# JoshEngels/RangeFilteredANN

Measured on AMD Instinct MI355X. Metric: QPS @ recall@10>=0.95, window fraction 2^-3, higher is better.
Workload: dtype f32

## Files before the change

### include/wann.h

```cpp
#ifndef WANN_H
#define WANN_H

#include <stdint.h>

#ifdef __cplusplus
extern "C" {
#endif

#define WANN_ABI_VERSION 5
#define WANN_MAX_DEGREE 128

enum { WANN_OK = 0, WANN_ERR_INVALID = 1, WANN_ERR_NO_DEVICE = 2, WANN_ERR_HIP = 3, WANN_ERR_IO = 4,
       WANN_ERR_UNSUPPORTED = 5 };

enum { WANN_METRIC_L2 = 0, WANN_METRIC_MIPS = 1 };
enum { WANN_DTYPE_F32 = 0, WANN_DTYPE_U8 = 1, WANN_DTYPE_I8 = 2, WANN_DTYPE_F16 = 3, WANN_DTYPE_BF16 = 5 };
enum {
  WANN_KIND_PREFILTER = 0,
  WANN_KIND_POSTFILTER = 1,
  WANN_KIND_TREE_PREFILTER = 2,
  WANN_KIND_TREE_VAMANA = 3,
  WANN_KIND_SUPER = 4
};

// ... 82 lines not shown
typedef struct {
  int64_t queries;
  int64_t unproven;
  int64_t rescued;
  int64_t groups;
  int64_t tiles;
  int64_t passes;
  int64_t handover_bytes;
} wann_dense_window_counters;
int wann_get_dense_window_counters(const wann_index *index, wann_dense_window_counters *out);

int64_t wann_set_exact_windows(wann_index *index, int64_t max_points);
typedef struct {
  int64_t queries;
  int64_t dense_queries;
  int64_t unproven;
  int64_t rescued;
  int64_t passes;
  int64_t rows_scanned;
} wann_exact_window_counters;
int wann_get_exact_window_counters(const wann_index *index, wann_exact_window_counters *out);

int64_t wann_num_points(const wann_index *index);
int64_t wann_dim(const wann_index *index);
int64_t wann_num_levels(const wann_index *index);
int64_t wann_level_size(const wann_index *index, int64_t level);
int wann_partition_range(const wann_index *index, int64_t level, int64_t idx, int64_t *start, int64_t *end);
int wann_partition_graph(const wann_index *index, int64_t level, int64_t idx, int32_t *rows, int64_t cap_rows,
                         int64_t max_degree);
int64_t wann_max_degree(const wann_index *index);
int64_t wann_device_bytes(const wann_index *index);

int wann_rows_fp16_exact(const float *rows, int64_t n, int64_t d);
int wann_set_half_rows(wann_index *index, int on);
int wann_half_rows(const wann_index *index);
int64_t wann_half_rows_bytes(const wann_index *index);
int wann_last_half_rows(const wann_index *index);
int wann_rows_u8_exact(const float *rows, int64_t n, int64_t d);
int64_t wann_byte_row_position(int64_t element);
int wann_set_byte_rows(wann_index *index, int on);
int wann_byte_rows(const wann_index *index);
int64_t wann_byte_rows_bytes(const wann_index *index);
int wann_last_byte_rows(const wann_index *index);
int wann_set_scan_rows(wann_index *index, int on);
int wann_scan_rows(const wann_index *index);
int wann_last_scan_rows(const wann_index *index);
int wann_num_replicas(const wann_index *index);

int wann_gather_layout(int64_t nq, int world, int shard, int64_t *lo, int64_t *count, int64_t *cap);
int wann_batch_search_allgather(wann_index *index, const void *queries, const float *ranges, int64_t nq, const char *method,
                                const wann_query_params *qp, int32_t **d_planes, int64_t *cap);

int wann_build_cache_shard(int kind, int metric, int dtype, const void *points, int64_t n, int64_t d,
                           const float *labels, int32_t cutoff, double split_factor,
                           double shift_factor, const wann_build_params *bp, int shard, int nshards,
                           int build_threads);

int wann_raw_beam_search(int metric, const float *points, int64_t n, int64_t d,
                         const int32_t *graph_rows , int64_t maxdeg,
                         int64_t subset_start, int64_t subset_n, const float *queries, int64_t nq,
                         const int64_t *query_ids, int64_t beam, int64_t limit,
                         int64_t degree_limit, int32_t *out_ids ,
                         float *out_dists , int32_t *out_sizes ,
                         int64_t *out_hops , int64_t *out_dist_cmps , int device);
int wann_raw_beam_search_typed(int metric, int dtype, const void *points, int64_t n, int64_t d,
                               const int32_t *graph_rows , int64_t maxdeg,
// ... 21 lines not shown
```

### rangefilteredann_amd/csrc/wann_abi.cpp

```cpp
#include "wann_host_internal.h"

struct wann_index::AsyncLane {
  Workspace ws;
  hipStream_t stream = nullptr, side = nullptr;
  hipEvent_t ready = nullptr;
  wann_counters last{};
  int last_store = kStoreRows;
  struct Job {
    const float *q, *r;
    int64_t nq, base;
    std::string method;
    wann_query_params qp;
    uint32_t *ids;
    float *dists;
    int64_t ticket;
    Tuning tune;
  };
  std::thread th;
  std::mutex m;
  std::condition_variable cv;
  bool has_job = false, busy = false, stop = false;
  Job job{};
  int64_t finished = -1;
  int rc = WANN_OK;
// ... 671 lines not shown
  return WANN_OK;
}
int64_t wann_max_degree(const wann_index *I) { return I ? I->H.spec.R : -1; }
int64_t wann_device_bytes(const wann_index *I) { return I ? I->device_bytes : -1; }

int wann_rows_fp16_exact(const float *rows, int64_t n, int64_t d) {
  if (n <= 0 || d <= 0) return 1;
  if (!rows) return 0;
  return rows_fp16_exact(rows, n, d, d, 0) ? 1 : 0;
}

int wann_set_half_rows(wann_index *I, int on) {
  if (!I) return -fail(WANN_ERR_INVALID, "null argument");
  int now;
  {
    std::lock_guard<std::mutex> lk(I->tune_mu);
    now = I->half_rows_on = on != 0 && I->d_half.p != nullptr;
  }
  for (auto &R : I->replicas) {
    std::lock_guard<std::mutex> lr(R->tune_mu);
    R->half_rows_on = on != 0 && R->d_half.p != nullptr;
  }
  return now;
}

int wann_half_rows(const wann_index *I) {
  if (!I) return 0;
  wann_index *M = const_cast<wann_index *>(I);
  std::lock_guard<std::mutex> lk(M->tune_mu);
  return I->half_rows_on ? 1 : 0;
}

int64_t wann_half_rows_bytes(const wann_index *I) { return I ? (int64_t)I->d_half.bytes() : -1; }
int wann_last_half_rows(const wann_index *I) { return I ? I->last_half_rows.load() : 0; }

int wann_rows_u8_exact(const float *rows, int64_t n, int64_t d) {
  if (n <= 0 || d <= 0) return 1;
  if (!rows) return 0;
  return rows_u8_exact(rows, n, d, d, 0) ? 1 : 0;
}

int64_t wann_byte_row_position(int64_t element) { return element < 0 ? -1 : u8_row_position(element); }

int wann_set_byte_rows(wann_index *I, int on) {
  if (!I) return -fail(WANN_ERR_INVALID, "null argument");
  int now;
  {
    std::lock_guard<std::mutex> lk(I->tune_mu);
    now = I->byte_rows_on = on != 0 && I->d_bytes.p != nullptr;
  }
  for (auto &R : I->replicas) {
    std::lock_guard<std::mutex> lr(R->tune_mu);
    R->byte_rows_on = on != 0 && R->d_bytes.p != nullptr;
  }
  return now;
}

int wann_byte_rows(const wann_index *I) {
  if (!I) return 0;
  wann_index *M = const_cast<wann_index *>(I);
  std::lock_guard<std::mutex> lk(M->tune_mu);
  return I->byte_rows_on ? 1 : 0;
}

int64_t wann_byte_rows_bytes(const wann_index *I) { return I ? (int64_t)I->d_bytes.bytes() : -1; }
int wann_last_byte_rows(const wann_index *I) { return I ? I->last_byte_rows.load() : 0; }
// ... 44 lines not shown
```

### rangefilteredann_amd/csrc/wann_build.cpp

```cpp
#include "wann_build.h"
#include "wann_device.h"
#include "wann_bf16.h"
#include "wann_half.h"

#include <algorithm>
#include <atomic>
#include <climits>
#include <cmath>
#include <condition_variable>
#include <cstdio>
#include <cstdlib>
#include <cstring>
#include <mutex>
#include <stdexcept>
#include <sys/stat.h>
#include <thread>
#include <unistd.h>
#include <chrono>

namespace wann {

namespace {
class WorkerPool {
 public:
// ... 128 lines not shown
    if (!exact.load(std::memory_order_relaxed)) return;
    const float *p = rows + r * stride;
    for (int64_t j = 0; j < d; j++) {
      uint32_t u = 0, v = 1;
      if (p[j] >= 0.f && p[j] <= 255.f) {
        const float back = (float)(uint8_t)p[j];
        memcpy(&u, p + j, 4);
        memcpy(&v, &back, 4);
      }
      if (u != v) {
        exact.store(false, std::memory_order_relaxed);
        return;
      }
    }
  });
  return exact.load();
}

void pack_u8_rows(const float *rows, int64_t n, int64_t d, int64_t stride, int64_t out_words, int threads, float *out) {
  parallel_for(n, threads > 0 ? threads : default_threads(), [&](int64_t r) {
    const float *src = rows + r * stride;
    uint8_t *dst = reinterpret_cast<uint8_t *>(out + r * out_words);
    for (int64_t j = 0; j < d; j++) dst[j] = (uint8_t)src[j];
  });
}

void interleave_u8_rows(float *rows, int64_t n, int64_t words, int threads) {
  if (words <= 0 || words % 8 != 0) throw std::runtime_error("interleave_u8_rows: a row is a whole number of 32-byte groups");
  parallel_for(n, threads > 0 ? threads : default_threads(), [&](int64_t r) {
    uint8_t *row = reinterpret_cast<uint8_t *>(rows + r * words);
    for (int64_t g = 0; g < words * 4; g += 32) {
      uint8_t t[32];
      for (int e = 0; e < 32; e++) t[u8_row_position(e)] = row[g + e];
      memcpy(row + g, t, 32);
    }
  });
}

static inline uint64_t mix64(uint64_t x) {
  x = (x ^ (x >> 30)) * UINT64_C(0xbf58476d1ce4e5b9);
  x = (x ^ (x >> 27)) * UINT64_C(0x94d049bb133111eb);
  return x ^ (x >> 31);
}

static inline float l2_ref_order(const float *a, const float *b, int d) {
  const int D8 = (d + 7) >> 3;
  float acc[8] = {0, 0, 0, 0, 0, 0, 0, 0};
  const bool odd = D8 & 1;
  for (int i = 0; i < D8; i++) {
    const int blk = odd ? (i == 0 ? D8 - 1 : i - 1) : i;
    const float *pa = a + 8 * blk, *pb = b + 8 * blk;
    for (int j = 0; j < 8; j++) {
      float t = pa[j] - pb[j];
      acc[j] = std::fmaf(t, t, acc[j]);
    }
  }
  return ((((((acc[0] + acc[1]) + acc[2]) + acc[3]) + acc[4]) + acc[5]) + acc[6]) + acc[7];
}

static inline float mips_ref_order(const float *p, const float *q, int d) {
  const int dv = d & ~7;
  float r = 0.f;
  for (int i = 0; i < dv; i++) {
    volatile float prod = q[i] * p[i];
    r = r + prod;
  }
// ... 622 lines not shown
```

### rangefilteredann_amd/csrc/wann_build.h

```cpp
#pragma once
#include <stdint.h>

#include <functional>
#include <string>
#include <vector>

namespace wann {

struct HostGraph {
  int64_t n = 0;
  int32_t maxdeg = 0;
  std::vector<int32_t> rows;
  int32_t *row(int64_t i) { return rows.data() + i * (maxdeg + 1); }
  const int32_t *row(int64_t i) const { return rows.data() + i * (maxdeg + 1); }
};

struct HostPart {
  int64_t start = 0, n = 0;
  float lo = 0, hi = 0;
  HostGraph g;
};

struct BuildSpec {
  int kind = 0, metric = 0;
  int dtype = 0;
  int64_t n = 0, d = 0, stride = 0;
  int32_t cutoff = 1000;
  double split_factor = 2, shift_factor = 0.5;
  int64_t R = 64, L = 500;
  double alpha = 1.0;
  std::string cache;
  int threads = 0;
};

struct HostIndex {
  BuildSpec spec;
  bool vamana_leaves = false, sorted = false;
  std::vector<float> pts;
  std::vector<float> labels;
  std::vector<uint32_t> decoding;
  std::vector<std::vector<int64_t>> offsets;
  std::vector<int64_t> sup_size, sup_shift;
  std::vector<std::vector<HostPart>> levels;
  std::vector<float> fv_sorted;
  std::vector<int32_t> fi_sorted;
};

void parallel_for(int64_t n, int threads, const std::function<void(int64_t)> &f);
int default_threads();

bool rows_fp16_exact(const float *rows, int64_t n, int64_t d, int64_t stride, int threads);
bool rows_u8_exact(const float *rows, int64_t n, int64_t d, int64_t stride, int threads);
void pack_u8_rows(const float *rows, int64_t n, int64_t d, int64_t stride, int64_t out_words, int threads, float *out);
void interleave_u8_rows(float *rows, int64_t n, int64_t words, int threads);

float host_distance(int metric, const float *p, const float *q, int d);

bool graph_file_load(const std::string &path, HostGraph &g);
bool graph_file_save(const std::string &path, const HostGraph &g);
std::string graph_file_name(const BuildSpec &s, float lo, float hi, int64_t n);

std::vector<int32_t> insertion_order(int64_t n);

void vamana_build(const float *pts, int64_t stride, int64_t d, int metric, int64_t start, int64_t n,
                  int64_t R, int64_t L, double alpha, HostGraph &g, int threads);

void build_host_index(HostIndex &H, const void *points, const float *labels, int shard = -1,
                      int nshards = 0, std::vector<HostPart *> *pending = nullptr);
void build_pending_on_host(HostIndex &H, std::vector<HostPart *> &pending);
void save_built_graphs(HostIndex &H, std::vector<HostPart *> &built, bool keep);

}
```

### rangefilteredann_amd/csrc/wann_device.h

```cpp
#pragma once
#include <stdint.h>

namespace wann {

struct PartDesc {
  int64_t row_base;
  int32_t start;
  int32_t n;
};

struct IndexView {
  const float *points;
  const float *labels;
  const uint32_t *decoding;
  const int32_t *graph;
  const PartDesc *parts;
  const float *fv_sorted;
  const int32_t *fi_sorted;
  const int64_t *wst_off;
  const int64_t *wst_ptr;
  const int64_t *level_part0;
  const int64_t *level_nb;
  const int64_t *sup_size;
  const int64_t *sup_shift;
  int64_t n;
  int32_t d, stride, rs, maxdeg, metric, kind, nlevels, cutoff, split, vamana_leaves;
  int32_t dtype;
};

constexpr bool two_byte_rows(int dtype) { return dtype == 3 || dtype == 5; }
constexpr int64_t two_byte_stride_words(int64_t d) { return ((d * 2 + 63) / 64) * 16; }

constexpr int kRowsU8Widened = 6;
constexpr int64_t u8_widened_stride_words(int64_t d) { return ((d + 63) / 64) * 16; }
constexpr int64_t u8_row_position(int64_t e) { return 32 * (e >> 5) + 16 * ((e >> 2) & 1) + 4 * ((e >> 3) & 3) + (e & 3); }
constexpr bool widened_rows(int dtype) { return two_byte_rows(dtype) || dtype == kRowsU8Widened; }

inline int query_words(const IndexView &v) { return widened_rows(v.dtype) ? ((v.d + 15) & ~15) : v.stride; }

enum { T_EMPTY = 0, T_GRAPH = 1, T_BRUTE = 2, T_BRUTE_GATHER = 3, T_PARENT = 4 };
constexpr int kTaskExactWindow = 32;
enum { M_OPTIMIZED = 0, M_THREE_SPLIT = 1, M_FENWICK = 2 };

struct Task {
  int32_t query;
  int32_t mode;
  int32_t part;
  int32_t flags;
  int64_t a, b;
  float lo, hi;
};

struct CoverCounters {
  unsigned long long queries, unproven, rescued, groups, tiles, passes, handover_bytes;
};

struct Counters {
  unsigned long long beam_searches, hops, dist_cmps, brute_rows, label_reads, unsupported;
  unsigned long long spec_searches, spec_hops, spec_dist_cmps;
  unsigned long long poll_timeouts;
  unsigned long long gemm_queries, gemm_unproven, gemm_rescued;
  unsigned long long deep_handoffs;
  unsigned long long lookaheads_used;
  unsigned long long big_searches, big_hops, packet_hops, own_scorings, prefetched_hops;
// ... 233 lines not shown
```

### rangefilteredann_amd/csrc/wann_host.cpp

```cpp
#include "wann_host_internal.h"
#include "wann_bf16.h"
#include "wann_half.h"

namespace wann_host {


thread_local std::string g_err;
int fail(int code, const std::string &msg) {
  g_err = msg;
  return code;
}

int usable_devices() {
  int n = 0;
  if (hipGetDeviceCount(&n) != hipSuccess) return 0;
  return n;
}

int hash_bits(int64_t beam) {
  return std::max<int>(10, (int)std::ceil(std::log2((double)(beam * beam))) - 2);
}

void convert_rows(const HostGraph &g, int rs, int32_t *out) {
  for (int64_t i = 0; i < g.n; i++) {
// ... 50 lines not shown
  v.maxdeg = (int32_t)s.R;
  v.rs = (int32_t)(((s.R + 15) / 16) * 16);
  v.nlevels = (int32_t)H.levels.size();

  if (two_byte_rows(s.dtype)) {
    std::vector<float> rows((size_t)s.n * v.stride, 0.f);
    parallel_for(s.n, s.threads > 0 ? s.threads : default_threads(), [&](int64_t r) {
      const float *src = H.pts.data() + r * s.stride;
      uint16_t *dst = reinterpret_cast<uint16_t *>(rows.data() + r * v.stride);
      for (int64_t j = 0; j < s.d; j++) dst[j] = float_to_two_byte(s.dtype, src[j]);
    });
    I.d_points.upload(rows);
  } else {
    I.d_points.upload(H.pts);
  }
  if (s.dtype == WANN_DTYPE_F32 && H.vamana_leaves && rows_fp16_exact(H.pts.data(), s.n, s.d, s.stride, s.threads)) {
    const int64_t hstride = ((s.d * 2 + 63) / 64) * 16;
    std::vector<float> rows;
    try {
      rows.assign((size_t)s.n * hstride, 0.f);
      I.d_half.ensure(rows.size());
    } catch (std::bad_alloc &) {
      I.d_half.release();
    } catch (HipError &) {
      (void)hipGetLastError();
      I.d_half.release();
    }
    if (I.d_half.p) {
      parallel_for(s.n, s.threads > 0 ? s.threads : default_threads(), [&](int64_t r) {
        const float *src = H.pts.data() + r * s.stride;
        uint16_t *dst = reinterpret_cast<uint16_t *>(rows.data() + r * hstride);
        for (int64_t j = 0; j < s.d; j++) dst[j] = float_to_half(src[j]);
      });
      I.d_half.upload(rows);
    }
  }
  if (s.dtype == WANN_DTYPE_F32 && H.vamana_leaves && rows_u8_exact(H.pts.data(), s.n, s.d, s.stride, s.threads)) {
    const int64_t bstride = u8_widened_stride_words(s.d);
    std::vector<float> rows;
    try {
      rows.assign((size_t)s.n * bstride, 0.f);
      I.d_bytes.ensure(rows.size());
    } catch (std::bad_alloc &) {
      I.d_bytes.release();
    } catch (HipError &) {
      (void)hipGetLastError();
      I.d_bytes.release();
    }
    if (I.d_bytes.p) {
      pack_u8_rows(H.pts.data(), s.n, s.d, s.stride, bstride, s.threads, rows.data());
      interleave_u8_rows(rows.data(), s.n, bstride, s.threads);
      I.d_bytes.upload(rows);
    }
  }
  I.d_labels.upload(H.labels);
  I.d_decoding.upload(H.decoding);
  v.points = I.d_points.p;
  v.labels = I.d_labels.p;
  v.decoding = I.d_decoding.p;
  if (s.kind == WANN_KIND_PREFILTER) {
    I.d_fv.upload(H.fv_sorted);
    I.d_fi.upload(H.fi_sorted);
    v.fv_sorted = I.d_fv.p;
    v.fi_sorted = I.d_fi.p;
  }
  int64_t rows = 0;
// ... 39 lines not shown
            for (int j = 0; j < deg; j++) {
              if (r[1 + j] < 0 || r[1 + j] >= P.n) throw std::runtime_error("graph edge out of range");
              o[j] = r[1 + j];
            }
            for (int j = deg; j < v.rs; j++) o[j] = -1;
          }
          HIP_CHECK(hipMemcpy(I.d_graph.p + (pd.row_base + r0) * v.rs, stage.data(), stage.size() * 4, hipMemcpyHostToDevice));
        }
      }
    v.graph = I.d_graph.p;
  }
  if (!H.offsets.empty()) {
    std::vector<int64_t> flat, ptr;
    for (auto &o : H.offsets) {
      ptr.push_back((int64_t)flat.size());
      flat.insert(flat.end(), o.begin(), o.end());
    }
    ptr.push_back((int64_t)flat.size());
    I.d_wst_off.upload(flat);
    I.d_wst_ptr.upload(ptr);
    v.wst_off = I.d_wst_off.p;
    v.wst_ptr = I.d_wst_ptr.p;
  }
  if (!H.sup_size.empty()) {
    I.d_sup_size.upload(H.sup_size);
    I.d_sup_shift.upload(H.sup_shift);
    v.sup_size = I.d_sup_size.p;
    v.sup_shift = I.d_sup_shift.p;
  }
  I.search_view = v;
  if (I.d_half.p) {
    I.search_view.points = I.d_half.p;
    I.search_view.stride = (int32_t)(((s.d * 2 + 63) / 64) * 16);
    I.search_view.dtype = WANN_DTYPE_F16;
    I.half_rows_on = true;
  }
  I.byte_view = v;
  if (I.d_bytes.p) {
    I.byte_view.points = I.d_bytes.p;
    I.byte_view.stride = (int32_t)u8_widened_stride_words(s.d);
    I.byte_view.dtype = kRowsU8Widened;
  }
  I.device_bytes = (int64_t)(I.d_points.bytes() + I.d_labels.bytes() + I.d_decoding.bytes() + I.d_graph.bytes() +
                             I.d_parts.bytes() + I.d_fv.bytes() + I.d_fi.bytes() + I.d_wst_off.bytes());
}

int ensure_filter_scratch(DevBuf<int32_t> &table, DevBuf<int32_t> &epoch, DevBuf<uint32_t> &seen, int64_t &layout, int slots,
                          int table_bits, int64_t seen_words, hipStream_t st, bool any_slots) {
  if (any_slots && layout > table_bits && layout < 32 && ((size_t)slots << layout) * sizeof(int32_t) <= ((size_t)20 << 30)) table_bits = (int)layout;
  const size_t need = (size_t)slots << table_bits;
  const int64_t want = any_slots ? (int64_t)table_bits : (((int64_t)slots << 8) | table_bits);
  const bool fresh = need > table.cap || (size_t)slots > epoch.cap;
  table.ensure(need);
  epoch.ensure((size_t)slots);
  seen.ensure((size_t)slots * (size_t)seen_words);
  if (fresh || layout != want) {
    HIP_CHECK(hipMemsetAsync(table.p, 0, table.cap * sizeof(int32_t), st));
    HIP_CHECK(hipMemsetAsync(epoch.p, 0, epoch.cap * sizeof(int32_t), st));
    layout = want;
  }
  return table_bits;
}

constexpr int kLdsGranule = 1280;
inline int lds_blocks_per_cu(int per_block) { return kLdsPerWorkgroup / (((per_block + kLdsGranule - 1) / kLdsGranule) * kLdsGranule); }

RoundCfg config_for(const wann_index &I, const IndexView &V, const Tuning &T, int64_t first_beam, int64_t cap, int64_t work_items, bool big_lds, bool force_table,
// ... 130 lines not shown
```

### rangefilteredann_amd/csrc/wann_kernels_body.inc

```
#include <hip/hip_runtime.h>
#include <stdint.h>

#include <algorithm>

#include "wann_device.h"
#include "wann_wave.h"

namespace wann {

#if WANN_DT == 0
#define WANN_DT_NS dt_f32
#elif WANN_DT == 1
#define WANN_DT_NS dt_u8
#elif WANN_DT == 2
#define WANN_DT_NS dt_i8
#elif WANN_DT == 3
#define WANN_DT_NS dt_f16
#elif WANN_DT == 5
#define WANN_DT_NS dt_bf16
#else
#define WANN_DT_NS dt_w8
#endif
#if WANN_DT == 3
#define WANN_DT_TPARAM , int ROWS_DT = 3
#elif WANN_DT == 5
#define WANN_DT_TPARAM , int ROWS_DT = 5
#elif WANN_DT == 6
#define WANN_DT_TPARAM , int ROWS_DT = 6
#else
#define WANN_DT_TPARAM
#endif
#ifndef WANN_MIPS_WAVES
#define WANN_MIPS_WAVES 3
#endif
namespace WANN_DT_NS {


__device__ __forceinline__ int hash_bits_dev(long long beam) {
  long long sq = beam * beam;
  int e = (sq <= 1) ? 0 : (64 - __builtin_clzll((unsigned long long)(sq - 1)));
  e -= 2;
  return e < 10 ? 10 : e;
}

__device__ __forceinline__ void la_withdraw(const SearchArgs &A, int la) {
  if (atomicExch(&A.par_done[la], 2) == 1) {
    atomicAdd(&A.ctr->spec_searches, 1ull);
    atomicAdd(&A.ctr->spec_hops, (unsigned long long)__hip_atomic_load(&A.sub_hops[la], __ATOMIC_RELAXED, __HIP_MEMORY_SCOPE_AGENT));
    atomicAdd(&A.ctr->spec_dist_cmps, (unsigned long long)__hip_atomic_load(&A.sub_cmps[la], __ATOMIC_RELAXED, __HIP_MEMORY_SCOPE_AGENT));
  }
  atomicCAS(A.dyn_list + A.next_beam[la], la, -2 - la);
}

__device__ __forceinline__ int la_slot_of(const SearchArgs &A, int t) {
  long long v = __hip_atomic_load(&A.sub_cmps[t], __ATOMIC_RELAXED, __HIP_MEMORY_SCOPE_AGENT);
  for (int spin = 0; v == -2 && spin < 4096; spin++) {
    __builtin_amdgcn_s_sleep(2);
    v = __hip_atomic_load(&A.sub_cmps[t], __ATOMIC_RELAXED, __HIP_MEMORY_SCOPE_AGENT);
  }
  return v < 0 ? -1 : (int)v;
}
// ... 1279 lines not shown
#endif
  dim3 grid(blocks), block(64 * kWavesPerBlock);
  return a.ix.metric == 1 ? launch_brute_t<1>(a, grid, block, lds, (hipStream_t)stream) : launch_brute_t<0>(a, grid, block, lds, (hipStream_t)stream);
}

}

#if WANN_DT == 0
namespace dt_u8 {
int launch_search(const SearchArgs &a, const LaunchCfg &cfg, void *stream);
int search_occupancy(const SearchArgs &a, const LaunchCfg &cfg);
int launch_brute(const BruteArgs &a, int blocks, void *stream);
}
namespace dt_i8 {
int launch_search(const SearchArgs &a, const LaunchCfg &cfg, void *stream);
int search_occupancy(const SearchArgs &a, const LaunchCfg &cfg);
int launch_brute(const BruteArgs &a, int blocks, void *stream);
}
namespace dt_f16 {
int launch_search(const SearchArgs &a, const LaunchCfg &cfg, void *stream);
int search_occupancy(const SearchArgs &a, const LaunchCfg &cfg);
int launch_brute(const BruteArgs &a, int blocks, void *stream);
}
namespace dt_bf16 {
int launch_search(const SearchArgs &a, const LaunchCfg &cfg, void *stream);
int search_occupancy(const SearchArgs &a, const LaunchCfg &cfg);
int launch_brute(const BruteArgs &a, int blocks, void *stream);
}
namespace dt_w8 {
int launch_search(const SearchArgs &a, const LaunchCfg &cfg, void *stream);
int search_occupancy(const SearchArgs &a, const LaunchCfg &cfg);
int launch_brute(const BruteArgs &a, int blocks, void *stream);
}
int search_occupancy(const SearchArgs &a, const LaunchCfg &cfg) {
  return a.ix.dtype == 1 ? dt_u8::search_occupancy(a, cfg) : a.ix.dtype == 2 ? dt_i8::search_occupancy(a, cfg)
       : a.ix.dtype == 3 ? dt_f16::search_occupancy(a, cfg) : a.ix.dtype == 5 ? dt_bf16::search_occupancy(a, cfg)
       : a.ix.dtype == kRowsU8Widened ? dt_w8::search_occupancy(a, cfg) : dt_f32::search_occupancy(a, cfg);
}
int launch_search(const SearchArgs &a, const LaunchCfg &cfg, void *stream) {
  return a.ix.dtype == 1 ? dt_u8::launch_search(a, cfg, stream) : a.ix.dtype == 2 ? dt_i8::launch_search(a, cfg, stream)
       : a.ix.dtype == 3 ? dt_f16::launch_search(a, cfg, stream) : a.ix.dtype == 5 ? dt_bf16::launch_search(a, cfg, stream)
       : a.ix.dtype == kRowsU8Widened ? dt_w8::launch_search(a, cfg, stream) : dt_f32::launch_search(a, cfg, stream);
}
int launch_brute(const BruteArgs &a, int blocks, void *stream) {
  return a.ix.dtype == 1 ? dt_u8::launch_brute(a, blocks, stream) : a.ix.dtype == 2 ? dt_i8::launch_brute(a, blocks, stream)
       : a.ix.dtype == 3 ? dt_f16::launch_brute(a, blocks, stream) : a.ix.dtype == 5 ? dt_bf16::launch_brute(a, blocks, stream)
       : a.ix.dtype == kRowsU8Widened ? dt_w8::launch_brute(a, blocks, stream) : dt_f32::launch_brute(a, blocks, stream);
}

int launch_finalize(const FinalizeArgs &a, void *stream) {
  if (a.nq == 0) return 0;
  if (a.maxt > 1) {
    const int per_wave = finalize_lds_bytes_per_wave(a.k);
    int blocks = (int)std::min<int64_t>(2048, (a.nq + kWavesPerBlock - 1) / kWavesPerBlock);
    hipLaunchKernelGGL(k_finalize_multi, dim3(blocks), dim3(64 * kWavesPerBlock), (size_t)per_wave * kWavesPerBlock,
                       (hipStream_t)stream, a);
  } else {
    int threads = 256;
    int blocks = (int)((a.nq * (int64_t)a.k + threads - 1) / threads);
    hipLaunchKernelGGL(k_finalize, dim3(blocks), dim3(threads), 0, (hipStream_t)stream, a);
  }
  return check(hipGetLastError());
}

#endif

}
```

### rangefilteredann_amd/csrc/wann_wave.h

```cpp
#pragma once
#include <hip/hip_runtime.h>
#include <stdint.h>

#include "wann_device.h"

namespace wann {

typedef unsigned long long u64;

#ifdef WANN_PHASE_PROFILE
#define WANN_PROF_PTR(p) (p)
#else
#define WANN_PROF_PTR(p) ((unsigned long long *)nullptr)
#endif

#define WANN_LIKELY(x) __builtin_expect(!!(x), 1)
#define WANN_UNLIKELY(x) __builtin_expect(!!(x), 0)

#define WAVE_SYNC()                                            \
  do {                                                         \
    __builtin_amdgcn_fence(__ATOMIC_SEQ_CST, "wavefront");     \
    __builtin_amdgcn_wave_barrier();                           \
  } while (0)

// ... 15 lines not shown
__device__ __forceinline__ T *uniptr(T *p) {
  return reinterpret_cast<T *>(uni64((long long)reinterpret_cast<uintptr_t>(p)));
}
__device__ __forceinline__ int ctz64(u64 m) { return __builtin_ctzll(m); }
__device__ __forceinline__ int popc64(u64 m) { return __builtin_popcountll(m); }
__device__ __forceinline__ u64 lanemask_lt() { return ((u64)1 << lane_id()) - 1; }

__device__ __forceinline__ int wave_ticket(int32_t *cursor) {
  int lane;
  asm volatile("v_mbcnt_lo_u32_b32 %0, -1, 0\n\tv_mbcnt_hi_u32_b32 %0, -1, %0" : "=v"(lane));
  int t = 0;
  if (lane == 0) t = atomicAdd(cursor, 1);
  return __builtin_amdgcn_readfirstlane(t);
}

__device__ __forceinline__ uint32_t fkey(float f) {
  uint32_t u = __float_as_uint(f);
  return (u & 0x80000000u) ? ~u : (u | 0x80000000u);
}
__device__ __forceinline__ float funkey(uint32_t k) {
  return __uint_as_float((k & 0x80000000u) ? (k ^ 0x80000000u) : ~k);
}

__device__ __forceinline__ u64 hash64_2(u64 x) {
  x = (x ^ (x >> 30)) * 0xbf58476d1ce4e5b9ull;
  x = (x ^ (x >> 27)) * 0x94d049bb133111ebull;
  return x ^ (x >> 31);
}

#ifndef WANN_DT
#define WANN_DT 0
#endif
#define WANN_BYTE_ROWS (WANN_DT == 1 || WANN_DT == 2)
#define WANN_HALF_ROWS (WANN_DT == 3 || WANN_DT == 5)
#define WANN_WIDENED_ROWS (WANN_HALF_ROWS || WANN_DT == 6)

#if WANN_DT == 3
typedef uint2 rowblk_t;
__device__ __forceinline__ float h2f(uint32_t bits) { return (float)__builtin_bit_cast(_Float16, (unsigned short)bits); }
__device__ __forceinline__ float4 h4_to_f4(uint2 w) {
  return make_float4(h2f(w.x & 0xffffu), h2f(w.x >> 16), h2f(w.y & 0xffffu), h2f(w.y >> 16));
}
#define ld_blk(prow, e) (*reinterpret_cast<const uint2 *>(reinterpret_cast<const unsigned short *>(prow) + (e)))
#define cvt_blk(w) h4_to_f4(w)
#elif WANN_DT == 5
typedef uint2 rowblk_t;
__device__ __forceinline__ float4 b4_to_f4(uint2 w) {
  return make_float4(__uint_as_float(w.x << 16), __uint_as_float(w.x & 0xffff0000u), __uint_as_float(w.y << 16),
                     __uint_as_float(w.y & 0xffff0000u));
}
#define ld_blk(prow, e) (*reinterpret_cast<const uint2 *>(reinterpret_cast<const unsigned short *>(prow) + (e)))
#define cvt_blk(w) b4_to_f4(w)
#elif WANN_DT == 6
typedef uint32_t rowblk_t;
typedef uint32_t u32x4 __attribute__((ext_vector_type(4)));
typedef u32x4 rowquad_t __attribute__((aligned(8)));
__device__ __forceinline__ float4 u4_to_f4(uint32_t w) {
  return make_float4((float)(w & 0xffu), (float)((w >> 8) & 0xffu), (float)((w >> 16) & 0xffu), (float)(w >> 24));
}
#define ld_quad(prow, c, h) (*reinterpret_cast<const rowquad_t *>(reinterpret_cast<const unsigned char *>(prow) + 32 * (c) + 16 * (h)))
__device__ __forceinline__ uint32_t quad_blk(const u32x4 &q, int i) { return i == 0 ? q.x : i == 1 ? q.y : i == 2 ? q.z : q.w; }
#define cvt_blk(w) u4_to_f4(w)
typedef u32x4 rowheld_t;
constexpr int kHeldBlks = 4;
#define held_blk(w, i) quad_blk(w, i)
#else
typedef float4 rowblk_t;
#define ld_blk(prow, e) (*reinterpret_cast<const float4 *>(prow + e))
#define cvt_blk(w) (w)
#endif
#ifndef held_blk
typedef rowblk_t rowheld_t;
constexpr int kHeldBlks = 1;
#define held_blk(w, i) (w)
#endif
__device__ __forceinline__ int qv_words(const IndexView &ix) { return WANN_WIDENED_ROWS ? ((ix.d + 15) & ~15) : ix.stride; }

__device__ __forceinline__ constexpr int l2_order(int i, int n) { return (n & 1) ? (i == 0 ? n - 1 : i - 1) : i; }
#define q_blk(qv, b, h) (*reinterpret_cast<const float4 *>((qv) + 8 * (b) + 4 * (h)))

template <int N>
using RowBlks = rowheld_t[N > 0 ? (N + kHeldBlks - 1) / kHeldBlks : 1];
#define row_blk(rb, b) cvt_blk(held_blk((rb)[(b) / kHeldBlks], (b) % kHeldBlks))

template <int N, int NBC = 0, bool LAST_FIRST = false>
__device__ __forceinline__ void row_blks_load(RowBlks<N> &rb, const float *__restrict__ prow, int h, int nblk = 0, int b0 = 0) {
#if WANN_DT == 6
#pragma unroll
  for (int c = 0; c < (N + 3) / 4; c++)
    if (NBC > 0 ? 4 * c < NBC : b0 + 4 * c < nblk) rb[c] = ld_quad(prow, (b0 >> 2) + c, h);
#else
#pragma unroll
  for (int i = 0; i < N; i++) {
    const int j = LAST_FIRST ? l2_order(i, NBC) : i;
    if (NBC > 0 ? j < NBC : b0 + j < nblk) rb[j] = ld_blk(prow, 8 * (b0 + j) + 4 * h);
  }
#endif
}

typedef float f32x2 __attribute__((ext_vector_type(2)));

__device__ __forceinline__ void l2_step(f32x2 &lo, f32x2 &hi, const float4 &p, const float4 &q) {
  f32x2 t0 = f32x2{p.x, p.y} - f32x2{q.x, q.y};
  f32x2 t1 = f32x2{p.z, p.w} - f32x2{q.z, q.w};
  lo = __builtin_elementwise_fma(t0, t0, lo);
  hi = __builtin_elementwise_fma(t1, t1, hi);
}
__device__ __forceinline__ void l2_step(float &a0, float &a1, float &a2, float &a3, const float4 &p, const float4 &q) {
  float t;
  t = p.x - q.x; a0 = fmaf(t, t, a0);
  t = p.y - q.y; a1 = fmaf(t, t, a1);
  t = p.z - q.z; a2 = fmaf(t, t, a2);
  t = p.w - q.w; a3 = fmaf(t, t, a3);
}

__device__ __forceinline__ float l2_reduce(const f32x2 &lo, const f32x2 &hi) {
  const float s = ((lo.x + lo.y) + hi.x) + hi.y;
  const float other = __shfl_xor(s, 1);
  return (((other + lo.x) + lo.y) + hi.x) + hi.y;
}

template <int NB>
__device__ __forceinline__ float l2_pair(const float *__restrict__ prow, const float *qv, int D8,
                                         int h, bool active) {
  float a0 = 0.f, a1 = 0.f, a2 = 0.f, a3 = 0.f;
  if (active) {
#if WANN_DT == 6
    const int nfull = D8 & ~1;
    if (D8 & 1) {
      const int b = D8 - 1;
      const u32x4 last = ld_quad(prow, b >> 2, h);
      const float4 q = q_blk(qv, b, h);
      l2_step(a0, a1, a2, a3, cvt_blk(quad_blk(last, b & 3)), q);
    }
    for (int b0 = 0; b0 < nfull; b0 += NB) {
      RowBlks<NB> buf;
      row_blks_load<NB>(buf, prow, h, nfull, b0);
#pragma unroll
      for (int j = 0; j < NB; j++)
        if (b0 + j < nfull) {
          const float4 q = q_blk(qv, b0 + j, h);
          l2_step(a0, a1, a2, a3, row_blk(buf, j), q);
        }
    }
#else
    for (int i0 = 0; i0 < D8; i0 += NB) {
      RowBlks<NB> buf;
#pragma unroll
      for (int j = 0; j < NB; j++)
        if (i0 + j < D8) buf[j] = ld_blk(prow, 8 * l2_order(i0 + j, D8) + 4 * h);
#pragma unroll
      for (int j = 0; j < NB; j++)
        if (i0 + j < D8) {
          const float4 q = q_blk(qv, l2_order(i0 + j, D8), h);
          l2_step(a0, a1, a2, a3, row_blk(buf, j), q);
        }
    }
#endif
  }
  return l2_reduce(f32x2{a0, a1}, f32x2{a2, a3});
}

template <int D8C>
__device__ __forceinline__ float l2_pair_ct(const float *__restrict__ prow, const float *qv, int h, bool active) {
  (void)active;
  RowBlks<D8C> buf;
// ... 2011 lines not shown
```

### rangefilteredann_amd/csrc/window_ann_pybind.cpp

```cpp
#include <pybind11/numpy.h>
#include <pybind11/pybind11.h>
#include <pybind11/stl.h>

#include <optional>
#include <stdexcept>
#include <string>
#include <vector>
#include <cstdio>

#include "../../include/wann.h"
#include "wann_bf16.h"

namespace py = pybind11;
using namespace pybind11::literals;

namespace wannpy {

struct BuildParams {
  long max_degree, limit;
  double alpha;
  std::string cache_path;
  BuildParams(long R, long L, double a, std::string c) : max_degree(R), limit(L), alpha(a), cache_path(std::move(c)) {}
};

// ... 523 lines not shown
  add_variant<WANN_METRIC_MIPS, WANN_DTYPE_F16>(m, "Float16Mips");
  add_variant<WANN_METRIC_L2, WANN_DTYPE_BF16>(m, "BFloat16Euclidian");
  add_variant<WANN_METRIC_MIPS, WANN_DTYPE_BF16>(m, "BFloat16Mips");

  add_vamana<WANN_METRIC_L2, WANN_DTYPE_F32>(m, "float_euclidian", "VamanaFloatEuclidianIndex");
  add_vamana<WANN_METRIC_MIPS, WANN_DTYPE_F32>(m, "float_mips", "VamanaFloatMipsIndex");
  add_vamana<WANN_METRIC_L2, WANN_DTYPE_U8>(m, "uint8_euclidian", "VamanaUInt8EuclidianIndex");
  add_vamana<WANN_METRIC_MIPS, WANN_DTYPE_U8>(m, "uint8_mips", "VamanaUInt8MipsIndex");
  add_vamana<WANN_METRIC_L2, WANN_DTYPE_I8>(m, "int8_euclidian", "VamanaInt8EuclidianIndex");
  add_vamana<WANN_METRIC_MIPS, WANN_DTYPE_I8>(m, "int8_mips", "VamanaInt8MipsIndex");

  for (const char *cls : {"PrefilterIndex", "RangeFilterTreeIndex", "PostfilterVamanaIndex", "VamanaRangeFilterTreeIndex",
                          "SuperOptimizedPostfilterTreeIndex"})
    for (const char *metric : {"Euclidian", "Mips"})
      m.attr((std::string(cls) + "Uint8" + metric).c_str()) = m.attr((std::string(cls) + "UInt8" + metric).c_str());

  m.def("bfloat16_bits", [](py::object a) {
    py::array b = bf16_bits_of(a);
    if (!b) throw std::runtime_error("bfloat16_bits: not convertible to a float32 array");
    return b;
  }, "a"_a);
  m.def("bfloat16_round", [](py::object a) {
    FArray f = FArray::ensure(a);
    if (!f) throw std::runtime_error("bfloat16_round: not convertible to a float32 array");
    py::array_t<float> out(std::vector<py::ssize_t>(f.shape(), f.shape() + f.ndim()));
    const float *src = f.data();
    float *dst = out.mutable_data();
    for (py::ssize_t i = 0, n = f.size(); i < n; i++) dst[i] = wann::bf16_to_float(wann::float_to_bf16(src[i]));
    return out;
  }, "a"_a);
  m.def("device_count", [] { return wann_device_count(); });
  m.def("abi_version", [] { return wann_abi_version(); });
  m.def("byte_row_position", [](int64_t e) { return wann_byte_row_position(e); }, py::arg("element"));
  m.def(
      "build_cache_shard",
      [](int kind, int metric, FArray points, FArray labels, int32_t cutoff, double split, double shift,
         const BuildParams &bp, int shard, int nshards, int threads) {
        if (points.ndim() != 2 || labels.ndim() != 1) throw std::runtime_error("bad shapes");
        wann_build_params wb{bp.max_degree, bp.limit, bp.alpha, bp.cache_path.c_str()};
        const float *pp = points.data();
        const float *lp = labels.data();
        int64_t n = points.shape(0), d = points.shape(1);
        int rc;
        {
          py::gil_scoped_release nogil;
          rc = wann_build_cache_shard(kind, metric, WANN_DTYPE_F32, pp, n, d, lp, cutoff, split, shift, &wb, shard,
                                      nshards, threads);
        }
        if (rc) raise_last("build_cache_shard failed");
      },
      "kind"_a, "metric"_a, "points"_a, "filter_values"_a, "cutoff"_a, "split_factor"_a, "shift_factor"_a,
      "build_params"_a, "shard"_a, "nshards"_a, "threads"_a = 0);
  m.def(
      "raw_beam_search",
      [](int metric, FArray points, py::array_t<int32_t, py::array::c_style | py::array::forcecast> graph_rows,
         int64_t subset_start, FArray queries, py::array_t<int64_t, py::array::c_style | py::array::forcecast> query_ids,
         int64_t beam, int64_t limit, int64_t degree_limit, int device) {
        if (points.ndim() != 2 || graph_rows.ndim() != 2 || queries.ndim() != 2) throw std::runtime_error("bad shapes");
        int64_t n = points.shape(0), d = points.shape(1), sn = graph_rows.shape(0), md = graph_rows.shape(1) - 1;
        int64_t nq = queries.shape(0);
        py::array_t<int32_t> ids({(size_t)nq, (size_t)beam});
        py::array_t<float> dists({(size_t)nq, (size_t)beam});
        py::array_t<int32_t> sizes((size_t)nq);
        py::array_t<int64_t> hops((size_t)nq), cmps((size_t)nq);
        int rc = wann_raw_beam_search(metric, points.data(), n, d, graph_rows.data(), md, subset_start, sn,
                                      queries.data(), nq, query_ids.data(), beam, limit, degree_limit,
// ... 35 lines not shown
```

Before: 3.871 million.

## Interleave fp16 rows so each lane loads paired 16-byte blocks

Adds a new fp16 row variant (dtype 7) whose elements are permuted on the host within each 32-byte group, so each half-wave lane reads one 16-byte vector per pair of 4-element blocks instead of separate 8-byte loads. The search view for half rows now points at this interleaved layout, and a dedicated kernel instantiation is added. The intent is fewer, wider global loads in the distance loop, at the cost of another kernel build and a host-side reshuffle during index build.

```diff
diff --git a/include/wann.h b/include/wann.h
--- a/include/wann.h
+++ b/include/wann.h
@@ -138,6 +138,7 @@
 int64_t wann_device_bytes(const wann_index *index);
 
 int wann_rows_fp16_exact(const float *rows, int64_t n, int64_t d);
+int64_t wann_half_row_position(int64_t element);
 int wann_set_half_rows(wann_index *index, int on);
 int wann_half_rows(const wann_index *index);
 int64_t wann_half_rows_bytes(const wann_index *index);
diff --git a/rangefilteredann_amd/csrc/wann_abi.cpp b/rangefilteredann_amd/csrc/wann_abi.cpp
--- a/rangefilteredann_amd/csrc/wann_abi.cpp
+++ b/rangefilteredann_amd/csrc/wann_abi.cpp
@@ -727,6 +727,8 @@
 }
 
 int64_t wann_half_rows_bytes(const wann_index *I) { return I ? (int64_t)I->d_half.bytes() : -1; }
+
+int64_t wann_half_row_position(int64_t element) { return element < 0 ? -1 : h16_row_position(element); }
 int wann_last_half_rows(const wann_index *I) { return I ? I->last_half_rows.load() : 0; }
 
 int wann_rows_u8_exact(const float *rows, int64_t n, int64_t d) {
diff --git a/rangefilteredann_amd/csrc/wann_build.cpp b/rangefilteredann_amd/csrc/wann_build.cpp
--- a/rangefilteredann_amd/csrc/wann_build.cpp
+++ b/rangefilteredann_amd/csrc/wann_build.cpp
@@ -184,6 +184,18 @@
     for (int64_t g = 0; g < words * 4; g += 32) {
       uint8_t t[32];
       for (int e = 0; e < 32; e++) t[u8_row_position(e)] = row[g + e];
+      memcpy(row + g, t, 32);
+    }
+  });
+}
+
+void interleave_h16_rows(float *rows, int64_t n, int64_t words, int threads) {
+  if (words <= 0 || words % 8 != 0) throw std::runtime_error("interleave_h16_rows: a row is a whole number of 32-byte groups");
+  parallel_for(n, threads > 0 ? threads : default_threads(), [&](int64_t r) {
+    uint16_t *row = reinterpret_cast<uint16_t *>(rows + r * words);
+    for (int64_t g = 0; g < words * 2; g += 16) {
+      uint16_t t[16];
+      for (int e = 0; e < 16; e++) t[h16_row_position(e)] = row[g + e];
       memcpy(row + g, t, 32);
     }
   });
diff --git a/rangefilteredann_amd/csrc/wann_build.h b/rangefilteredann_amd/csrc/wann_build.h
--- a/rangefilteredann_amd/csrc/wann_build.h
+++ b/rangefilteredann_amd/csrc/wann_build.h
@@ -53,6 +53,7 @@
 bool rows_u8_exact(const float *rows, int64_t n, int64_t d, int64_t stride, int threads);
 void pack_u8_rows(const float *rows, int64_t n, int64_t d, int64_t stride, int64_t out_words, int threads, float *out);
 void interleave_u8_rows(float *rows, int64_t n, int64_t words, int threads);
+void interleave_h16_rows(float *rows, int64_t n, int64_t words, int threads);
 
 float host_distance(int metric, const float *p, const float *q, int d);
 
diff --git a/rangefilteredann_amd/csrc/wann_device.h b/rangefilteredann_amd/csrc/wann_device.h
--- a/rangefilteredann_amd/csrc/wann_device.h
+++ b/rangefilteredann_amd/csrc/wann_device.h
@@ -28,8 +28,10 @@
   int32_t dtype;
 };
 
-constexpr bool two_byte_rows(int dtype) { return dtype == 3 || dtype == 5; }
+constexpr int kRowsF16Paired = 7;
+constexpr bool two_byte_rows(int dtype) { return dtype == 3 || dtype == 5 || dtype == kRowsF16Paired; }
 constexpr int64_t two_byte_stride_words(int64_t d) { return ((d * 2 + 63) / 64) * 16; }
+constexpr int64_t h16_row_position(int64_t e) { return 16 * (e >> 4) + 8 * ((e >> 2) & 1) + 4 * ((e >> 3) & 1) + (e & 3); }
 
 constexpr int kRowsU8Widened = 6;
 constexpr int64_t u8_widened_stride_words(int64_t d) { return ((d + 63) / 64) * 16; }
diff --git a/rangefilteredann_amd/csrc/wann_host.cpp b/rangefilteredann_amd/csrc/wann_host.cpp
--- a/rangefilteredann_amd/csrc/wann_host.cpp
+++ b/rangefilteredann_amd/csrc/wann_host.cpp
@@ -106,6 +106,7 @@
         uint16_t *dst = reinterpret_cast<uint16_t *>(rows.data() + r * hstride);
         for (int64_t j = 0; j < s.d; j++) dst[j] = float_to_half(src[j]);
       });
+      interleave_h16_rows(rows.data(), s.n, hstride, s.threads);
       I.d_half.upload(rows);
     }
   }
@@ -211,7 +212,7 @@
   if (I.d_half.p) {
     I.search_view.points = I.d_half.p;
     I.search_view.stride = (int32_t)(((s.d * 2 + 63) / 64) * 16);
-    I.search_view.dtype = WANN_DTYPE_F16;
+    I.search_view.dtype = kRowsF16Paired;
     I.half_rows_on = true;
   }
   I.byte_view = v;
diff --git a/rangefilteredann_amd/csrc/wann_kernels_body.inc b/rangefilteredann_amd/csrc/wann_kernels_body.inc
--- a/rangefilteredann_amd/csrc/wann_kernels_body.inc
+++ b/rangefilteredann_amd/csrc/wann_kernels_body.inc
@@ -18,6 +18,8 @@
 #define WANN_DT_NS dt_f16
 #elif WANN_DT == 5
 #define WANN_DT_NS dt_bf16
+#elif WANN_DT == 7
+#define WANN_DT_NS dt_h16
 #else
 #define WANN_DT_NS dt_w8
 #endif
@@ -27,6 +29,8 @@
 #define WANN_DT_TPARAM , int ROWS_DT = 5
 #elif WANN_DT == 6
 #define WANN_DT_TPARAM , int ROWS_DT = 6
+#elif WANN_DT == 7
+#define WANN_DT_TPARAM , int ROWS_DT = 7
 #else
 #define WANN_DT_TPARAM
 #endif
@@ -1372,20 +1376,28 @@
 int search_occupancy(const SearchArgs &a, const LaunchCfg &cfg);
 int launch_brute(const BruteArgs &a, int blocks, void *stream);
 }
+namespace dt_h16 {
+int launch_search(const SearchArgs &a, const LaunchCfg &cfg, void *stream);
+int search_occupancy(const SearchArgs &a, const LaunchCfg &cfg);
+int launch_brute(const BruteArgs &a, int blocks, void *stream);
+}
 int search_occupancy(const SearchArgs &a, const LaunchCfg &cfg) {
   return a.ix.dtype == 1 ? dt_u8::search_occupancy(a, cfg) : a.ix.dtype == 2 ? dt_i8::search_occupancy(a, cfg)
        : a.ix.dtype == 3 ? dt_f16::search_occupancy(a, cfg) : a.ix.dtype == 5 ? dt_bf16::search_occupancy(a, cfg)
-       : a.ix.dtype == kRowsU8Widened ? dt_w8::search_occupancy(a, cfg) : dt_f32::search_occupancy(a, cfg);
+       : a.ix.dtype == kRowsU8Widened ? dt_w8::search_occupancy(a, cfg) : a.ix.dtype == kRowsF16Paired ? dt_h16::search_occupancy(a, cfg)
+       : dt_f32::search_occupancy(a, cfg);
 }
 int launch_search(const SearchArgs &a, const LaunchCfg &cfg, void *stream) {
   return a.ix.dtype == 1 ? dt_u8::launch_search(a, cfg, stream) : a.ix.dtype == 2 ? dt_i8::launch_search(a, cfg, stream)
        : a.ix.dtype == 3 ? dt_f16::launch_search(a, cfg, stream) : a.ix.dtype == 5 ? dt_bf16::launch_search(a, cfg, stream)
-       : a.ix.dtype == kRowsU8Widened ? dt_w8::launch_search(a, cfg, stream) : dt_f32::launch_search(a, cfg, stream);
+       : a.ix.dtype == kRowsU8Widened ? dt_w8::launch_search(a, cfg, stream) : a.ix.dtype == kRowsF16Paired ? dt_h16::launch_search(a, cfg, stream)
+       : dt_f32::launch_search(a, cfg, stream);
 }
 int launch_brute(const BruteArgs &a, int blocks, void *stream) {
   return a.ix.dtype == 1 ? dt_u8::launch_brute(a, blocks, stream) : a.ix.dtype == 2 ? dt_i8::launch_brute(a, blocks, stream)
        : a.ix.dtype == 3 ? dt_f16::launch_brute(a, blocks, stream) : a.ix.dtype == 5 ? dt_bf16::launch_brute(a, blocks, stream)
-       : a.ix.dtype == kRowsU8Widened ? dt_w8::launch_brute(a, blocks, stream) : dt_f32::launch_brute(a, blocks, stream);
+       : a.ix.dtype == kRowsU8Widened ? dt_w8::launch_brute(a, blocks, stream) : a.ix.dtype == kRowsF16Paired ? dt_h16::launch_brute(a, blocks, stream)
+       : dt_f32::launch_brute(a, blocks, stream);
 }
 
 int launch_finalize(const FinalizeArgs &a, void *stream) {
diff --git a/rangefilteredann_amd/csrc/wann_kernels_h16.hip b/rangefilteredann_amd/csrc/wann_kernels_h16.hip
--- /dev/null
+++ b/rangefilteredann_amd/csrc/wann_kernels_h16.hip
@@ -0,0 +1,2 @@
+#define WANN_DT 7
+#include "wann_kernels_body.inc"
diff --git a/rangefilteredann_amd/csrc/wann_wave.h b/rangefilteredann_amd/csrc/wann_wave.h
--- a/rangefilteredann_amd/csrc/wann_wave.h
+++ b/rangefilteredann_amd/csrc/wann_wave.h
@@ -71,7 +71,7 @@
 #define WANN_DT 0
 #endif
 #define WANN_BYTE_ROWS (WANN_DT == 1 || WANN_DT == 2)
-#define WANN_HALF_ROWS (WANN_DT == 3 || WANN_DT == 5)
+#define WANN_HALF_ROWS (WANN_DT == 3 || WANN_DT == 5 || WANN_DT == 7)
 #define WANN_WIDENED_ROWS (WANN_HALF_ROWS || WANN_DT == 6)
 
 #if WANN_DT == 3
@@ -81,6 +81,15 @@
   return make_float4(h2f(w.x & 0xffffu), h2f(w.x >> 16), h2f(w.y & 0xffffu), h2f(w.y >> 16));
 }
 #define ld_blk(prow, e) (*reinterpret_cast<const uint2 *>(reinterpret_cast<const unsigned short *>(prow) + (e)))
+#define cvt_blk(w) h4_to_f4(w)
+#elif WANN_DT == 7
+typedef uint2 rowblk_t;
+typedef uint32_t u32x4 __attribute__((ext_vector_type(4)));
+__device__ __forceinline__ float h2f(uint32_t bits) { return (float)__builtin_bit_cast(_Float16, (unsigned short)bits); }
+__device__ __forceinline__ float4 h4_to_f4(uint2 w) {
+  return make_float4(h2f(w.x & 0xffffu), h2f(w.x >> 16), h2f(w.y & 0xffffu), h2f(w.y >> 16));
+}
+#define ld_pair(prow, c, h) (*reinterpret_cast<const u32x4 *>(reinterpret_cast<const unsigned char *>(prow) + 32 * (c) + 16 * (h)))
 #define cvt_blk(w) h4_to_f4(w)
 #elif WANN_DT == 5
 typedef uint2 rowblk_t;
@@ -128,6 +137,14 @@
 #pragma unroll
   for (int c = 0; c < (N + 3) / 4; c++)
     if (NBC > 0 ? 4 * c < NBC : b0 + 4 * c < nblk) rb[c] = ld_quad(prow, (b0 >> 2) + c, h);
+#elif WANN_DT == 7
+#pragma unroll
+  for (int c = 0; c < (N + 1) / 2; c++)
+    if (NBC > 0 ? 2 * c < NBC : b0 + 2 * c < nblk) {
+      const u32x4 p = ld_pair(prow, (b0 >> 1) + c, h);
+      rb[2 * c] = make_uint2(p.x, p.y);
+      if (2 * c + 1 < N) rb[2 * c + 1] = make_uint2(p.z, p.w);
+    }
 #else
 #pragma unroll
   for (int i = 0; i < N; i++) {
@@ -164,13 +181,19 @@
                                          int h, bool active) {
   float a0 = 0.f, a1 = 0.f, a2 = 0.f, a3 = 0.f;
   if (active) {
-#if WANN_DT == 6
+#if WANN_DT == 6 || WANN_DT == 7
     const int nfull = D8 & ~1;
     if (D8 & 1) {
       const int b = D8 - 1;
+#if WANN_DT == 6
       const u32x4 last = ld_quad(prow, b >> 2, h);
       const float4 q = q_blk(qv, b, h);
       l2_step(a0, a1, a2, a3, cvt_blk(quad_blk(last, b & 3)), q);
+#else
+      const u32x4 last = ld_pair(prow, b >> 1, h);
+      const float4 q = q_blk(qv, b, h);
+      l2_step(a0, a1, a2, a3, cvt_blk(make_uint2(last.x, last.y)), q);
+#endif
     }
     for (int b0 = 0; b0 < nfull; b0 += NB) {
       RowBlks<NB> buf;
diff --git a/rangefilteredann_amd/csrc/window_ann_pybind.cpp b/rangefilteredann_amd/csrc/window_ann_pybind.cpp
--- a/rangefilteredann_amd/csrc/window_ann_pybind.cpp
+++ b/rangefilteredann_amd/csrc/window_ann_pybind.cpp
@@ -579,6 +579,7 @@
   m.def("device_count", [] { return wann_device_count(); });
   m.def("abi_version", [] { return wann_abi_version(); });
   m.def("byte_row_position", [](int64_t e) { return wann_byte_row_position(e); }, py::arg("element"));
+  m.def("half_row_position", [](int64_t e) { return wann_half_row_position(e); }, py::arg("element"));
   m.def(
       "build_cache_shard",
       [](int kind, int metric, FArray points, FArray labels, int32_t cutoff, double split, double shift,
```

New measurement: 4.182 million (median of 6 runs). +8.0%, better.
